# khanhptnk/magical-1

Hardware: AMD Instinct MI355X
Metric: env-steps/sec (whole node) at N instances/GPU, 1/2/4/8 MI355X (higher is better)
Workload: dtype f64

## Files before the change

magical-1_amd/csrc/mg_step.h:

```cpp
#pragma once
#include "mg_phys.h"
#include "mg_prof.h"

struct BodyR { int b; double minv, iinv; };
MG_DEV BodyR bodyr(const MGState &S, int e, int b) {
    if (b < 0) return {b, 0.0, 0.0};
    return {b, AT(S.bminv, b), AT(S.biinv, b)};
}
MG_DEV V2 bv(const MGState &S, int e, int b) { return b < 0 ? v2(0.0, 0.0) : v2(AT(S.bvx, b), AT(S.bvy, b)); }
MG_DEV double bwv(const MGState &S, int e, int b) { return b < 0 ? 0.0 : AT(S.bw, b); }
MG_DEV V2 bvb(const MGState &S, int e, int b) { return b < 0 ? v2(0.0, 0.0) : v2(AT(S.bvbx, b), AT(S.bvby, b)); }
MG_DEV double bwb(const MGState &S, int e, int b) { return b < 0 ? 0.0 : AT(S.bwb, b); }
MG_DEV V2 bp(const MGState &S, int e, int b) { return b < 0 ? v2(0.0, 0.0) : v2(AT(S.bpx, b), AT(S.bpy, b)); }
MG_DEV double ban(const MGState &S, int e, int b) { return b < 0 ? 0.0 : AT(S.ba, b); }

MG_DEV void apply_impulse(const MGState &S, int e, const BodyR &B, V2 j, V2 r) {
    if (B.b < 0) return;
    AT(S.bvx, B.b) = AT(S.bvx, B.b) + j.x * B.minv;
    AT(S.bvy, B.b) = AT(S.bvy, B.b) + j.y * B.minv;
    AT(S.bw, B.b) += B.iinv * vcross(r, j);
}
MG_DEV void apply_impulses(const MGState &S, int e, const BodyR &A, const BodyR &B, V2 r1, V2 r2, V2 j) {
    apply_impulse(S, e, A, vneg(j), r1);
    apply_impulse(S, e, B, j, r2);
// ... 227 lines not shown
    AT(S.au, slot) = u_a * u_b;
    AT(S.asa, slot) = sa_body; AT(S.asb, slot) = sb_body;
    if (AT(S.astate, slot) == ARB_CACHED) AT(S.astate, slot) = ARB_FIRST;
    int na_ = S.nactive[e];
    if (na_ < S.arb_cap) { AT(S.active, na_) = slot; S.nactive[e] = na_ + 1; }
    else S.overflow[e] |= 1;
    AT(S.astamp, slot) = S.stamp[e];
}

MG_DEV void arbiter_update(const MGState &S, const mg_library *L, int e, int key, const ShapeW &A, const ShapeW &B,
                           double ua, double ub, const Collision &info) {
    arbiter_update_t(S, L, e, key, A.type, A.body, B.type, B.body, ua, ub, info);
}

MG_DEV void arbiter_prestep(const MGState &S, const mg_library *L, int e, int slot, double dt) {
    int a = AT(S.asa, slot), b = AT(S.asb, slot);
    BodyR A = bodyr(S, e, a), B = bodyr(S, e, b);
    V2 n = v2(AT(S.anx, slot), AT(S.any, slot));
    V2 body_delta = vsub(bp(S, e, b), bp(S, e, a));
    int cnt = AT(S.acount, slot);
    for (int k = 0; k < cnt; k++) {
        V2 r1 = v2(ACON(k, AC_R1X, slot), ACON(k, AC_R1Y, slot)), r2 = v2(ACON(k, AC_R2X, slot), ACON(k, AC_R2Y, slot));
        ACON(k, AC_NMASS, slot) = 1.0 / (k_scalar_body(A, r1, n) + k_scalar_body(B, r2, n));
        V2 pn = vperp(n);
        ACON(k, AC_TMASS, slot) = 1.0 / (k_scalar_body(A, r1, pn) + k_scalar_body(B, r2, pn));
        double dist = vdot(vadd(vsub(r2, r1), body_delta), n);
        ACON(k, AC_BIAS, slot) = -L->collision_bias_coef * cpmin(0.0, dist + L->slop) / dt;
        ACON(k, AC_JB, slot) = 0.0;
    }
}

MG_DEV void arbiter_cached(const MGState &S, int e, int slot, double dt_coef) {
    if (AT(S.astate, slot) == ARB_FIRST) return;
    int a = AT(S.asa, slot), b = AT(S.asb, slot);
    BodyR A = bodyr(S, e, a), B = bodyr(S, e, b);
    V2 n = v2(AT(S.anx, slot), AT(S.any, slot));
    int cnt = AT(S.acount, slot);
    for (int k = 0; k < cnt; k++) {
        V2 j = vrotate(n, v2(ACON(k, AC_JN, slot), ACON(k, AC_JT, slot)));
        apply_impulses(S, e, A, B, v2(ACON(k, AC_R1X, slot), ACON(k, AC_R1Y, slot)),
                       v2(ACON(k, AC_R2X, slot), ACON(k, AC_R2Y, slot)), vmult(j, dt_coef));
    }
}

MG_DEV void arbiter_apply(const MGState &S, int e, int slot) {
    int a = AT(S.asa, slot), b = AT(S.asb, slot);
    BodyR A = bodyr(S, e, a), B = bodyr(S, e, b);
    V2 n = v2(AT(S.anx, slot), AT(S.any, slot));
    double friction = AT(S.au, slot);
    int cnt = AT(S.acount, slot);
    for (int k = 0; k < cnt; k++) {
        double nMass = ACON(k, AC_NMASS, slot);
        V2 r1 = v2(ACON(k, AC_R1X, slot), ACON(k, AC_R1Y, slot)), r2 = v2(ACON(k, AC_R2X, slot), ACON(k, AC_R2Y, slot));
        V2 vb1 = vadd(bvb(S, e, a), vmult(vperp(r1), bwb(S, e, a)));
        V2 vb2 = vadd(bvb(S, e, b), vmult(vperp(r2), bwb(S, e, b)));
        V2 vr = relative_velocity(S, e, a, b, r1, r2);
        double vbn = vdot(vsub(vb2, vb1), n);
        double vrn = vdot(vr, n);
        double vrt = vdot(vr, vperp(n));
        double jbn = (ACON(k, AC_BIAS, slot) - vbn) * nMass;
        double jbnOld = ACON(k, AC_JB, slot);
        double jBias = cpmax(jbnOld + jbn, 0.0);
        ACON(k, AC_JB, slot) = jBias;
        double jn = -(0.0 + vrn) * nMass;
        double jnOld = ACON(k, AC_JN, slot);
        double jnAcc = cpmax(jnOld + jn, 0.0);
        ACON(k, AC_JN, slot) = jnAcc;
        double jtMax = friction * jnAcc;
        double jt = -vrt * ACON(k, AC_TMASS, slot);
        double jtOld = ACON(k, AC_JT, slot);
        double jtAcc = cpclamp(jtOld + jt, -jtMax, jtMax);
        ACON(k, AC_JT, slot) = jtAcc;
        V2 jb = vmult(n, jBias - jbnOld);
        apply_bias_impulse(S, e, A, vneg(jb), r1);
        apply_bias_impulse(S, e, B, jb, r2);
        apply_impulses(S, e, A, B, r1, r2, vrotate(n, v2(jnAcc - jnOld, jtAcc - jtOld)));
    }
}

template <int NB>
struct RegBodies { double vx[NB], vy[NB], w[NB], vbx[NB], vby[NB], wb[NB], minv[NB], iinv[NB]; };

struct RegCons {
    double r1x, r1y, r2x, r2y, k11, k12, k21, k22, bias, bias2, jacc, jacc2, jmax, ratio, ratio_inv, isum, rate, twrn,
        wcoef;
};

template <int NB>
MG_DEV void rapply(RegBodies<NB> &R, int b, V2 j, V2 r) {
    if (b < 0) return;
    R.vx[b] = R.vx[b] + j.x * R.minv[b];
    R.vy[b] = R.vy[b] + j.y * R.minv[b];
    R.w[b] += R.iinv[b] * vcross(r, j);
}
template <int NB> MG_DEV V2 rv(const RegBodies<NB> &R, int b) { return b < 0 ? v2(0.0, 0.0) : v2(R.vx[b], R.vy[b]); }
template <int NB> MG_DEV double rw(const RegBodies<NB> &R, int b) { return b < 0 ? 0.0 : R.w[b]; }
template <int NB> MG_DEV double rii(const RegBodies<NB> &R, int b) { return b < 0 ? 0.0 : R.iinv[b]; }

template <int NB>
MG_DEV void rb_load(RegBodies<NB> &R, const MGState &S, int e) {
#pragma unroll
    for (int b = 0; b < NB; b++) {
        R.vx[b] = AT(S.bvx, b); R.vy[b] = AT(S.bvy, b); R.w[b] = AT(S.bw, b);
        R.vbx[b] = AT(S.bvbx, b); R.vby[b] = AT(S.bvby, b); R.wb[b] = AT(S.bwb, b);
        R.minv[b] = AT(S.bminv, b); R.iinv[b] = AT(S.biinv, b);
    }
}
template <int NB>
MG_DEV void rb_store(const RegBodies<NB> &R, const MGState &S, int e) {
#pragma unroll
    for (int b = 0; b < NB; b++) {
        AT(S.bvx, b) = R.vx[b]; AT(S.bvy, b) = R.vy[b]; AT(S.bw, b) = R.w[b];
        AT(S.bvbx, b) = R.vbx[b]; AT(S.bvby, b) = R.vby[b]; AT(S.bwb, b) = R.wb[b];
    }
}

MG_DEV void rc_load(RegCons &q, const MGState &S, int e, int c, int type, double dt) {
    q.jacc = CPA(CP_JACC, c); q.jacc2 = 0.0; q.jmax = CPA(CP_MAXF, c) * dt;
    q.isum = CPA(CP_ISUM, c); q.bias = CPA(CP_BIAS, c);
    if (type == MG_C_PIVOT) {
        q.jacc2 = CPA(CP_JACC2, c); q.bias2 = CPA(CP_BIAS2, c);
        q.r1x = CPA(CP_R1X, c); q.r1y = CPA(CP_R1Y, c); q.r2x = CPA(CP_R2X, c); q.r2y = CPA(CP_R2Y, c);
        q.k11 = CPA(CP_K11, c); q.k12 = CPA(CP_K12, c); q.k21 = CPA(CP_K21, c); q.k22 = CPA(CP_K22, c);
    }
    if (type == MG_C_GEAR) { q.ratio = CPA(CP_RATIO, c); q.ratio_inv = CPA(CP_RATIO_INV, c); }
    if (type == MG_C_MOTOR) q.rate = CPA(CP_RATE, c);
    if (type == MG_C_SPRING) { q.twrn = CPA(CP_TWRN, c); q.wcoef = CPA(CP_WCOEF, c); }
}
MG_DEV void rc_store(const RegCons &q, const MGState &S, int e, int c, int type) {
    CPA(CP_JACC, c) = q.jacc;
    if (type == MG_C_PIVOT) CPA(CP_JACC2, c) = q.jacc2;
    if (type == MG_C_SPRING) CPA(CP_TWRN, c) = q.twrn;
}

template <int NB>
MG_DEV void rcons_cached(RegBodies<NB> &R, const RegCons &q, int a, int b, int type, double dt_coef) {
    switch (type) {
    case MG_C_PIVOT: {
        V2 j = vmult(v2(q.jacc, q.jacc2), dt_coef);
        rapply(R, a, vneg(j), v2(q.r1x, q.r1y));
        rapply(R, b, j, v2(q.r2x, q.r2y));
        break;
    }
    case MG_C_GEAR: {
        double j = q.jacc * dt_coef;
        if (a >= 0) R.w[a] -= j * R.iinv[a] * q.ratio_inv;
        if (b >= 0) R.w[b] += j * R.iinv[b];
        break;
    }
    case MG_C_ROTLIMIT:
    case MG_C_MOTOR: {
        double j = q.jacc * dt_coef;
        if (a >= 0) R.w[a] -= j * R.iinv[a];
        if (b >= 0) R.w[b] += j * R.iinv[b];
        break;
    }
    default: break;
    }
}

template <int NB>
MG_DEV void rcons_apply(RegBodies<NB> &R, RegCons &q, int a, int b, int type) {
    switch (type) {
    case MG_C_PIVOT: {
        V2 r1 = v2(q.r1x, q.r1y), r2 = v2(q.r2x, q.r2y);
        V2 v1 = vadd(rv(R, a), vmult(vperp(r1), rw(R, a)));
        V2 v2_ = vadd(rv(R, b), vmult(vperp(r2), rw(R, b)));
        V2 vr = vsub(v2_, v1);
        V2 d = vsub(v2(q.bias, q.bias2), vr);
        V2 j = v2(d.x * q.k11 + d.y * q.k12, d.x * q.k21 + d.y * q.k22);
        V2 jOld = v2(q.jacc, q.jacc2);
        V2 jAcc = vclamp(vadd(jOld, j), q.jmax);
        q.jacc = jAcc.x; q.jacc2 = jAcc.y;
        V2 dj = vsub(jAcc, jOld);
        rapply(R, a, vneg(dj), r1);
        rapply(R, b, dj, r2);
        break;
    }
    case MG_C_GEAR: {
        double wr = rw(R, b) * q.ratio - rw(R, a);
        double j = (q.bias - wr) * q.isum;
        double jOld = q.jacc;
        double jAcc = cpclamp(jOld + j, -q.jmax, q.jmax);
        q.jacc = jAcc;
        j = jAcc - jOld;
        if (a >= 0) R.w[a] -= j * R.iinv[a] * q.ratio_inv;
        if (b >= 0) R.w[b] += j * R.iinv[b];
        break;
    }
    case MG_C_ROTLIMIT: {
        double bias = q.bias;
        if (!bias) return;
        double wr = rw(R, b) - rw(R, a);
        double j = -(bias + wr) * q.isum;
        double jOld = q.jacc;
        double jAcc = bias < 0.0 ? cpclamp(jOld + j, 0.0, q.jmax) : cpclamp(jOld + j, -q.jmax, 0.0);
        q.jacc = jAcc;
        j = jAcc - jOld;
        if (a >= 0) R.w[a] -= j * R.iinv[a];
        if (b >= 0) R.w[b] += j * R.iinv[b];
        break;
    }
    case MG_C_MOTOR: {
        double wr = rw(R, b) - rw(R, a) + q.rate;
        double j = -wr * q.isum;
        double jOld = q.jacc;
        double jAcc = cpclamp(jOld + j, -q.jmax, q.jmax);
        q.jacc = jAcc;
        j = jAcc - jOld;
        if (a >= 0) R.w[a] -= j * R.iinv[a];
        if (b >= 0) R.w[b] += j * R.iinv[b];
        break;
    }
    case MG_C_SPRING: {
        double wrn = rw(R, a) - rw(R, b);
        double w_damp = (q.twrn - wrn) * q.wcoef;
        q.twrn = wrn + w_damp;
        double j_damp = w_damp * q.isum;
        q.jacc += j_damp;
        if (a >= 0) R.w[a] += j_damp * R.iinv[a];
        if (b >= 0) R.w[b] -= j_damp * R.iinv[b];
        break;
    }
    }
}

__host__ __device__ constexpr bool shape_body_slot(int k) { return k == 0 || k == 4 || k == 5 || k == 6; }
template <int NB>
struct ArbBody { bool m[NB]; };
template <int NB>
MG_DEV ArbBody<NB> arb_body(int b) {
    ArbBody<NB> h;
#pragma unroll
    for (int k = 0; k < NB; k++) h.m[k] = shape_body_slot(k) && b == k;
    return h;
}
template <int NB>
MG_DEV double hsel(const double (&x)[NB], const ArbBody<NB> &h) {
    double r = 0.0;
#pragma unroll
    for (int k = 0; k < NB; k++)
        if (shape_body_slot(k)) r = h.m[k] ? x[k] : r;
    return r;
}
template <int NB>
MG_DEV void hput(double (&x)[NB], const ArbBody<NB> &h, double v) {
#pragma unroll
    for (int k = 0; k < NB; k++)
        if (shape_body_slot(k)) x[k] = h.m[k] ? v : x[k];
}
template <int NB>
MG_DEV void happly(RegBodies<NB> &R, const ArbBody<NB> &h, double minv, double iinv, V2 j, V2 r) {
    hput(R.vx, h, hsel(R.vx, h) + j.x * minv);
    hput(R.vy, h, hsel(R.vy, h) + j.y * minv);
    hput(R.w, h, hsel(R.w, h) + iinv * vcross(r, j));
}
template <int NB>
MG_DEV void happly_bias(RegBodies<NB> &R, const ArbBody<NB> &h, double minv, double iinv, V2 j, V2 r) {
    hput(R.vbx, h, hsel(R.vbx, h) + j.x * minv);
    hput(R.vby, h, hsel(R.vby, h) + j.y * minv);
    hput(R.wb, h, hsel(R.wb, h) + iinv * vcross(r, j));
}
template <int NB>
MG_DEV void harb_cached(RegBodies<NB> &R, const MGState &S, int e, int slot, double dt_coef) {
    if (AT(S.astate, slot) == ARB_FIRST) return;
    const ArbBody<NB> ha = arb_body<NB>(AT(S.asa, slot)), hb = arb_body<NB>(AT(S.asb, slot));
    const double am = hsel(R.minv, ha), ai = hsel(R.iinv, ha), bm = hsel(R.minv, hb), bi = hsel(R.iinv, hb);
    V2 n = v2(AT(S.anx, slot), AT(S.any, slot));
    int cnt = AT(S.acount, slot);
    for (int k = 0; k < cnt; k++) {
        V2 j = vmult(vrotate(n, v2(ACON(k, AC_JN, slot), ACON(k, AC_JT, slot))), dt_coef);
        happly(R, ha, am, ai, vneg(j), v2(ACON(k, AC_R1X, slot), ACON(k, AC_R1Y, slot)));
        happly(R, hb, bm, bi, j, v2(ACON(k, AC_R2X, slot), ACON(k, AC_R2Y, slot)));
    }
}
template <int NB>
MG_DEV void harb_apply(RegBodies<NB> &R, const MGState &S, int e, int slot) {
    const int sa = AT(S.asa, slot), sb = AT(S.asb, slot);
    const ArbBody<NB> ha = arb_body<NB>(sa), hb = arb_body<NB>(sb);
    const double am = hsel(R.minv, ha), ai = hsel(R.iinv, ha), bm = hsel(R.minv, hb), bi = hsel(R.iinv, hb);
    const bool wa = __ballot(sa >= 0) != 0, wb = __ballot(sb >= 0) != 0;
    V2 n = v2(AT(S.anx, slot), AT(S.any, slot));
    double friction = AT(S.au, slot);
    int cnt = AT(S.acount, slot);
    for (int k = 0; k < cnt; k++) {
        double nMass = ACON(k, AC_NMASS, slot);
        V2 r1 = v2(ACON(k, AC_R1X, slot), ACON(k, AC_R1Y, slot)), r2 = v2(ACON(k, AC_R2X, slot), ACON(k, AC_R2Y, slot));
        V2 vb1 = v2(0.0, 0.0), v1 = v2(0.0, 0.0), vb2 = v2(0.0, 0.0), v2_ = v2(0.0, 0.0);
        if (wa) {
            vb1 = vadd(v2(hsel(R.vbx, ha), hsel(R.vby, ha)), vmult(vperp(r1), hsel(R.wb, ha)));
            v1 = vadd(v2(hsel(R.vx, ha), hsel(R.vy, ha)), vmult(vperp(r1), hsel(R.w, ha)));
        }
        if (wb) {
            vb2 = vadd(v2(hsel(R.vbx, hb), hsel(R.vby, hb)), vmult(vperp(r2), hsel(R.wb, hb)));
            v2_ = vadd(v2(hsel(R.vx, hb), hsel(R.vy, hb)), vmult(vperp(r2), hsel(R.w, hb)));
        }
        V2 vr = vsub(v2_, v1);
        double vbn = vdot(vsub(vb2, vb1), n);
        double vrn = vdot(vr, n);
        double vrt = vdot(vr, vperp(n));
        double jbn = (ACON(k, AC_BIAS, slot) - vbn) * nMass;
        double jbnOld = ACON(k, AC_JB, slot);
// ... 154 lines not shown
        if (k < a.cnt) { ACON(k, AC_JB, slot) = a.jb[k]; ACON(k, AC_JN, slot) = a.jn[k]; ACON(k, AC_JT, slot) = a.jt[k]; }
}
template <int NB, int A, int B>
MG_DEV void rarb_apply_k(RegBodies<NB> &R, RegArb &a) {
    const double am = A >= 0 ? R.minv[A] : 0.0, ai = A >= 0 ? R.iinv[A] : 0.0;
    const double bm = B >= 0 ? R.minv[B] : 0.0, bi = B >= 0 ? R.iinv[B] : 0.0;
    const V2 n = v2(a.nx, a.ny);
#pragma unroll
    for (int k = 0; k < 2; k++) {
        if (k >= a.cnt) break;
        const double nMass = a.nm[k];
        V2 r1 = v2(a.r1x[k], a.r1y[k]), r2 = v2(a.r2x[k], a.r2y[k]);
        V2 vb1 = v2(0.0, 0.0), v1 = v2(0.0, 0.0), vb2 = v2(0.0, 0.0), v2_ = v2(0.0, 0.0);
        if constexpr (A >= 0) {
            vb1 = vadd(v2(R.vbx[A], R.vby[A]), vmult(vperp(r1), R.wb[A]));
            v1 = vadd(v2(R.vx[A], R.vy[A]), vmult(vperp(r1), R.w[A]));
        }
        if constexpr (B >= 0) {
            vb2 = vadd(v2(R.vbx[B], R.vby[B]), vmult(vperp(r2), R.wb[B]));
            v2_ = vadd(v2(R.vx[B], R.vy[B]), vmult(vperp(r2), R.w[B]));
        }
        V2 vr = vsub(v2_, v1);
        double vbn = vdot(vsub(vb2, vb1), n);
        double vrn = vdot(vr, n);
        double vrt = vdot(vr, vperp(n));
        double jbn = (a.bias[k] - vbn) * nMass;
        double jbnOld = a.jb[k];
        double jBias = cpmax(jbnOld + jbn, 0.0);
        a.jb[k] = jBias;
        double jn = -(0.0 + vrn) * nMass;
        double jnOld = a.jn[k];
        double jnAcc = cpmax(jnOld + jn, 0.0);
        a.jn[k] = jnAcc;
        double jtMax = a.fr * jnAcc;
        double jt = -vrt * a.tm[k];
        double jtOld = a.jt[k];
        double jtAcc = cpclamp(jtOld + jt, -jtMax, jtMax);
        a.jt[k] = jtAcc;
        V2 jb = vmult(n, jBias - jbnOld);
        if constexpr (A >= 0) {
            const V2 m = vneg(jb);
            R.vbx[A] = R.vbx[A] + m.x * am; R.vby[A] = R.vby[A] + m.y * am; R.wb[A] = R.wb[A] + ai * vcross(r1, m);
        }
        if constexpr (B >= 0) {
            R.vbx[B] = R.vbx[B] + jb.x * bm; R.vby[B] = R.vby[B] + jb.y * bm; R.wb[B] = R.wb[B] + bi * vcross(r2, jb);
        }
        V2 j = vrotate(n, v2(jnAcc - jnOld, jtAcc - jtOld));
        if constexpr (A >= 0) {
            const V2 m = vneg(j);
            R.vx[A] = R.vx[A] + m.x * am; R.vy[A] = R.vy[A] + m.y * am; R.w[A] = R.w[A] + ai * vcross(r1, m);
        }
        if constexpr (B >= 0) {
            R.vx[B] = R.vx[B] + j.x * bm; R.vy[B] = R.vy[B] + j.y * bm; R.w[B] = R.w[B] + bi * vcross(r2, j);
        }
    }
}
template <int NB>
MG_DEV void rarb_row(RegBodies<NB> &R, RegArb &a) {
    switch (a.code) {
    case 0: rarb_apply_k<NB, 0, -1>(R, a); break;
    case 1: rarb_apply_k<NB, -1, 4>(R, a); break;
    case 2: rarb_apply_k<NB, -1, 5>(R, a); break;
    default:
        if constexpr (NB > 6) {
            switch (a.code) {
            case 3: rarb_apply_k<NB, -1, 6>(R, a); break;
            case 4: rarb_apply_k<NB, 0, 6>(R, a); break;
            case 5: rarb_apply_k<NB, 4, 6>(R, a); break;
            default: rarb_apply_k<NB, 5, 6>(R, a); break;
            }
        }
        break;
    }
}

template <int NCS, int C = 0>
MG_DEV void rstatic_load(RegCons *q, const MGState &S, int e, double dt) {
    if constexpr (C < NCS) {
        rc_load(q[C], S, e, C, static_cons(C).type, dt);
        rstatic_load<NCS, C + 1>(q, S, e, dt);
    }
}
template <int NCS, int C = 0>
MG_DEV void rstatic_store(const RegCons *q, const MGState &S, int e) {
    if constexpr (C < NCS) {
        rc_store(q[C], S, e, C, static_cons(C).type);
        rstatic_store<NCS, C + 1>(q, S, e);
    }
}
template <int NCS, int NB, int C = 0>
MG_DEV void rstatic_cached(RegBodies<NB> &R, const RegCons *q, double dt_coef) {
    if constexpr (C < NCS) {
        constexpr ConsDesc d = static_cons(C);
        rcons_cached(R, q[C], d.a, d.b, d.type, dt_coef);
        rstatic_cached<NCS, NB, C + 1>(R, q, dt_coef);
    }
}
template <int NCS, int NB, int C = 0>
MG_DEV void rstatic_apply(RegBodies<NB> &R, RegCons *q) {
    if constexpr (C < NCS) {
        constexpr ConsDesc d = static_cons(C);
        rcons_apply(R, q[C], d.a, d.b, d.type);
        rstatic_apply<NCS, NB, C + 1>(R, q);
    }
}

__host__ __device__ constexpr int static_nbodies(int ncs) { return ncs > 10 ? 7 : 6; }

template <int NCS, int NARB>
MG_DEV void static_solve(const MGState &S, int e, double dt, double dt_coef, int nact, MGProf &P) {
    constexpr int NB = static_nbodies(NCS);
    RegBodies<NB> R;
    RegCons q[NCS];
    rb_load(R, S, e);
    rstatic_load<NCS>(q, S, e, dt);
    for (int i = 0; i < nact; i++) harb_cached_row(R, S, e, AT(S.active, i), dt_coef);
    rstatic_cached<NCS>(R, q, dt_coef);
    MG_PP(P, 5);
    RegArb ra[NARB > 0 ? NARB : 1];
    int nreg = 0;
    if constexpr (NARB > 0) {
#pragma unroll
        for (int i = 0; i < NARB; i++) {
            ra[i].code = -1; ra[i].cnt = 0;
            if (i < nact) rarb_load(ra[i], S, e, AT(S.active, i));
        }
        bool ok = true;
#pragma unroll
        for (int i = 0; i < NARB; i++) {
            if (i < nact && ok && ra[i].code >= 0 && (NB > 6 || ra[i].code <= 2)) nreg = i + 1;
            else ok = false;
        }
    }
#pragma unroll 1
    for (int it = 0; it < MG_ITERATIONS; it++) {
        if constexpr (NARB > 0) {
#pragma unroll
            for (int i = 0; i < NARB; i++)
                if (i < nreg) rarb_row(R, ra[i]);
        }
        for (int i = nreg; i < nact; i++) harb_row(R, S, e, AT(S.active, i));
        rstatic_apply<NCS>(R, q);
    }
    if constexpr (NARB > 0) {
#pragma unroll
        for (int i = 0; i < NARB; i++)
            if (i < nreg) rarb_store(ra[i], S, e, AT(S.active, i));
    }
    rb_store(R, S, e);
    rstatic_store<NCS>(q, S, e);
}

MG_DEV void space_step(const MGState &S, const mg_library *L, int e, double dt, MGProf &P) {
    uint32_t stamp = S.stamp[e] + 1;
    S.stamp[e] = stamp;
    double prev_dt = S.curr_dt[e];
    S.curr_dt[e] = dt;
    int nact = S.nactive[e];
    for (int i = 0; i < nact; i++) AT(S.astate, AT(S.active, i)) = ARB_NORMAL;
    S.nactive[e] = 0;
    int nb = S.nbodies[e];
    for (int b = 0; b < nb; b++) {
        AT(S.bpx, b) = AT(S.bpx, b) + (AT(S.bvx, b) + AT(S.bvbx, b)) * dt;
        AT(S.bpy, b) = AT(S.bpy, b) + (AT(S.bvy, b) + AT(S.bvby, b)) * dt;
        body_set_angle_step(S, e, b, AT(S.ba, b) + (AT(S.bw, b) + AT(S.bwb, b)) * dt);
        AT(S.bvbx, b) = 0.0; AT(S.bvby, b) = 0.0; AT(S.bwb, b) = 0.0;
    }
    int ns = S.nshapes[e];
    for (int k = 0; k < ns; k++) shape_update_bb(S, L, e, k);
    MG_PP(P, 1);
    ShapeW A, W, B;
    for (int i = 0; i < ns; i++) {
        const double al = AT(S.sbbl, i), ab = AT(S.sbbb, i), ar = AT(S.sbbr, i), at = AT(S.sbbt, i);
        bool have_a = false;
        const int gi = AT(S.sgroup, i), bi = AT(S.sbody, i);
        const double ui = AT(S.su, i);
        for (int w = 0; w < 4 && !(gi & MG_GROUP_OFF); w++) {
            double wl, wb, wr, wt;
            wall_bb(w, wl, wb, wr, wt);
            if (!(al <= wr && wl <= ar && ab <= wt && wb <= at)) continue;
            if (!have_a) { load_shape(S, L, e, i, (uint64_t)AT(S.shash, i), A); have_a = true; }
            load_wall(w, W);
            Collision info;
            collide(A, W, info);
            if (info.count) arbiter_update(S, L, e, i * 128 + 100 + w, A, W, ui, 0.8, info);
        }
        for (int j = i + 1; j < ns; j++) {
            if (!(al <= AT(S.sbbr, j) && AT(S.sbbl, j) <= ar && ab <= AT(S.sbbt, j) && AT(S.sbbb, j) <= at))
                continue;
            if (AT(S.sbody, j) == bi) continue;
            int gj = AT(S.sgroup, j);
            if ((gi != 0 && gi == gj) || ((gi | gj) & MG_GROUP_OFF)) continue;
            if (surely_apart(S, L, e, i, j)) continue;
            if (!have_a) { load_shape(S, L, e, i, (uint64_t)AT(S.shash, i), A); have_a = true; }
            load_shape(S, L, e, j, (uint64_t)AT(S.shash, j), B);
            Collision info;
            collide(A, B, info);
            if (info.count) arbiter_update(S, L, e, i * 128 + j, A, B, ui, AT(S.su, j), info);
        }
    }
    MG_PP(P, 2);
    for (int i = 0; i < S.arb_cap; i++) {
        if (AT(S.akey, i) < 0) continue;
        uint32_t ticks = stamp - AT(S.astamp, i);
        if (ticks >= 1 && AT(S.astate, i) != ARB_CACHED) AT(S.astate, i) = ARB_CACHED;
        if (ticks >= 3) { AT(S.akey, i) = -1; AT(S.acount, i) = 0; }
    }
    MG_PP(P, 3);
    nact = S.nactive[e];
    int nc = S.ncons[e];
    for (int i = 0; i < nact; i++) arbiter_prestep(S, L, e, AT(S.active, i), dt);
    for (int c = 0; c < nc; c++) cons_prestep(S, e, c, dt);
    MG_PP(P, 4);
    double dt_coef = (prev_dt == 0.0 ? 0.0 : dt / prev_dt);
    for (int i = 0; i < nact; i++) arbiter_cached(S, e, AT(S.active, i), dt_coef);
    for (int c = 0; c < nc; c++) cons_cached(S, e, c, dt_coef);
    MG_PP(P, 5);
    for (int it = 0; it < MG_ITERATIONS; it++) {
        for (int i = 0; i < nact; i++) arbiter_apply(S, e, AT(S.active, i));
        for (int c = 0; c < nc; c++) cons_apply(S, e, c, dt);
    }
    MG_PP(P, 6);
}

MG_DEV double rl_d(double v, int src) {
    const uint64_t u = (uint64_t)__double_as_longlong(v);
    const uint32_t lo = (uint32_t)__builtin_amdgcn_readlane((int)(uint32_t)u, src);
    const uint32_t hi = (uint32_t)__builtin_amdgcn_readlane((int)(uint32_t)(u >> 32), src);
    return __longlong_as_double((long long)(((uint64_t)hi << 32) | lo));
}
MG_DEV uint64_t rl_u64(uint64_t v, int src) {
    const uint32_t lo = (uint32_t)__builtin_amdgcn_readlane((int)(uint32_t)v, src);
    const uint32_t hi = (uint32_t)__builtin_amdgcn_readlane((int)(uint32_t)(v >> 32), src);
// ... 736 lines not shown
```

magical-1_amd/csrc/mg_stepq.h:

```cpp
#pragma once
#include "mg_step.h"

template <int QL> MG_DEV int qlane(int ev, int s) { return ev * QL + s; }

MG_DEV double qshfl(double v, int src) {
    const uint64_t u = __double_as_longlong(v);
    const uint32_t lo = (uint32_t)__shfl((int)(uint32_t)u, src, 64), hi = (uint32_t)__shfl((int)(uint32_t)(u >> 32), src, 64);
    return __longlong_as_double((long long)(((uint64_t)hi << 32) | lo));
}
MG_DEV uint64_t qshfl_u64(uint64_t u, int src) {
    const uint32_t lo = (uint32_t)__shfl((int)(uint32_t)u, src, 64), hi = (uint32_t)__shfl((int)(uint32_t)(u >> 32), src, 64);
    return ((uint64_t)hi << 32) | lo;
}

template <int NC, int QL, int C = 0>
MG_DEV void static_prestep_quad(const MGState &S, int e, int sub, double dt) {
    if constexpr (C < NC) {
        constexpr ConsDesc d = static_cons(C);
        constexpr int owner = d.type == MG_C_SPRING ? 0 : C % QL;
        if (sub == owner) cons_prestep_impl(S, e, C, d.a, d.b, d.type, dt);
        static_prestep_quad<NC, QL, C + 1>(S, e, sub, dt);
    }
}

MG_DEV int quad_body(int p, int nb) {
    if (p == 0) return 0;
    if (p == 1) return 4;
    if (p == 2) return 5;
    if (nb == 7) return p == 3 ? 6 : p - 3;
    return p - 2;
}

MG_DEV uint64_t qshfl_xor_u64(uint64_t u, int m) {
    const uint32_t lo = (uint32_t)__shfl_xor((int)(uint32_t)u, m, 64), hi = (uint32_t)__shfl_xor((int)(uint32_t)(u >> 32), m, 64);
    return ((uint64_t)hi << 32) | lo;
}

MG_DEV bool quad_candidate(const MGState &S, const mg_library *L, int e, int i, int k) {
    const double al = AT(S.sbbl, i), ab = AT(S.sbbb, i), ar = AT(S.sbbr, i), at = AT(S.sbbt, i);
    const int gi = AT(S.sgroup, i);
    if (k < 4) {
        if (gi & MG_GROUP_OFF) return false;
        double wl, wb, wr, wt;
        wall_bb(k, wl, wb, wr, wt);
        return al <= wr && wl <= ar && ab <= wt && wb <= at;
    }
    const int j = i + 1 + (k - 4), gj = AT(S.sgroup, j);
    return al <= AT(S.sbbr, j) && AT(S.sbbl, j) <= ar && ab <= AT(S.sbbt, j) && AT(S.sbbb, j) <= at &&
           AT(S.sbody, j) != AT(S.sbody, i) && !((gi != 0 && gi == gj) || ((gi | gj) & MG_GROUP_OFF)) &&
           !surely_apart(S, L, e, i, j);
}

template <int NCS, int QL>
MG_DEV void narrowphase_quad(const MGState &S, const mg_library *L, int e, int sub, int ns) {
    ShapeW A, B;
    const int ntot = 4 * ns + (ns * (ns - 1)) / 2;
    for (int w0 = 0; w0 < ntot; w0 += 64) {
        const int wn = ntot - w0 < 64 ? ntot - w0 : 64;
        uint64_t hits = 0;
        {
            int i = 0, k = w0 + sub;
            while (i < ns && k >= 4 + ns - 1 - i) { k -= 4 + ns - 1 - i; i++; }
            for (int c = sub; c < wn; c += QL) {
                if (quad_candidate(S, L, e, i, k)) hits |= 1ull << c;
                k += QL;
                while (i < ns && k >= 4 + ns - 1 - i) { k -= 4 + ns - 1 - i; i++; }
            }
        }
#pragma unroll
        for (int off = 1; off < QL; off <<= 1)
            hits |= qshfl_xor_u64(hits, off);
        while (hits) {
            uint64_t rest = hits;
            int mine = -1;
#pragma unroll
            for (int q = 0; q < QL; q++) {
                if (!rest) break;
                const int b = __ffsll((long long)rest) - 1;
                rest &= rest - 1;
                if (q == sub) mine = b;
            }
            hits = rest;
            Collision info;
            info.count = 0;
            int key = 0, ta = 0, bi = 0, tb = 0, bb = -1;
            double ui = 0.0, ub = 0.0;
            if (mine >= 0) {
                int i = 0, k = w0 + mine;
                while (k >= 4 + ns - 1 - i) { k -= 4 + ns - 1 - i; i++; }
                bi = AT(S.sbody, i); ui = AT(S.su, i);
                ta = AT(S.spoly, i) < 0 ? WS_CIRCLE : WS_POLY;
                load_shape(S, L, e, i, (uint64_t)AT(S.shash, i), A);
                if (k < 4) {
                    load_wall(k, B);
                    key = i * 128 + 100 + k; ub = 0.8; tb = WS_SEGMENT; bb = -1;
                } else {
                    const int j = i + 1 + (k - 4);
                    load_shape(S, L, e, j, (uint64_t)AT(S.shash, j), B);
                    key = i * 128 + j; ub = AT(S.su, j); tb = B.type; bb = B.body;
                }
                collide(A, B, info);
            }
            const uint64_t bal = __ballot(info.count > 0);
            uint32_t m = 0;
#pragma unroll
            for (int s = 0; s < QL; s++) m |= (uint32_t)((bal >> qlane<QL>(e, s)) & 1ull) << s;
            for (int s = 0; s < QL; s++) {
                if (!((m >> s) & 1u)) continue;
                const int src = qlane<QL>(e, s);
                Collision q;
                q.count = __shfl(info.count, src, 64);
                q.n = v2(qshfl(info.n.x, src), qshfl(info.n.y, src));
#pragma unroll
                for (int kk = 0; kk < 2; kk++) {
                    q.p1[kk] = v2(qshfl(info.p1[kk].x, src), qshfl(info.p1[kk].y, src));
                    q.p2[kk] = v2(qshfl(info.p2[kk].x, src), qshfl(info.p2[kk].y, src));
                    q.hash[kk] = qshfl_u64(info.hash[kk], src);
                }
                const int qkey = __shfl(key, src, 64), qta = __shfl(ta, src, 64), qbi = __shfl(bi, src, 64);
                const int qtb = __shfl(tb, src, 64), qbb = __shfl(bb, src, 64);
                const double qui = qshfl(ui, src), qub = qshfl(ub, src);
                if (sub == 0) arbiter_update_t(S, L, e, qkey, qta, qbi, qtb, qbb, qui, qub, q);
            }
        }
    }
}

template <int NCS, int QL>
MG_DEV void space_step_quad(const MGState &S, const mg_library *L, int e, int sub, double dt, MGProf &P) {
    __syncthreads();
    const double prev_dt = S.curr_dt[e];
    const uint32_t stamp = S.stamp[e] + 1;
    const int nact0 = S.nactive[e], nb = S.nbodies[e], ns = S.nshapes[e];
    for (int i = sub; i < nact0; i += QL) AT(S.astate, AT(S.active, i)) = ARB_NORMAL;
    for (int p = sub; p < nb; p += QL) {
        const int b = quad_body(p, nb);
        AT(S.bpx, b) = AT(S.bpx, b) + (AT(S.bvx, b) + AT(S.bvbx, b)) * dt;
        AT(S.bpy, b) = AT(S.bpy, b) + (AT(S.bvy, b) + AT(S.bvby, b)) * dt;
        body_set_angle_step(S, e, b, AT(S.ba, b) + (AT(S.bw, b) + AT(S.bwb, b)) * dt);
        AT(S.bvbx, b) = 0.0; AT(S.bvby, b) = 0.0; AT(S.bwb, b) = 0.0;
    }
    __syncthreads();
    if (sub == 0) { S.stamp[e] = stamp; S.curr_dt[e] = dt; S.nactive[e] = 0; }
    for (int k = sub; k < ns; k += QL) shape_update_bb(S, L, e, k);
    __syncthreads();
    MG_PP(P, 1);
    narrowphase_quad<NCS, QL>(S, L, e, sub, ns);
    __syncthreads();
    MG_PP(P, 2);
    for (int i = sub; i < S.arb_cap; i += QL) {
        if (AT(S.akey, i) < 0) continue;
        const uint32_t ticks = stamp - AT(S.astamp, i);
        if (ticks >= 1 && AT(S.astate, i) != ARB_CACHED) AT(S.astate, i) = ARB_CACHED;
        if (ticks >= 3) { AT(S.akey, i) = -1; AT(S.acount, i) = 0; }
    }
    __syncthreads();
    MG_PP(P, 3);
    const int nact = S.nactive[e];
    for (int i = sub; i < nact; i += QL) arbiter_prestep(S, L, e, AT(S.active, i), dt);
    static_prestep_quad<NCS, QL>(S, e, sub, dt);
    __syncthreads();
    MG_PP(P, 4);
    const double dt_coef = (prev_dt == 0.0 ? 0.0 : dt / prev_dt);
    if (sub == 0) static_solve<NCS, (QL >= 8 ? 1 : 0)>(S, e, dt, dt_coef, nact, P);
    MG_PP(P, 6);
}

template <int NCS, int QL>
__device__ __forceinline__ void env_substeps_quad(const MGState &V, const mg_library *L, int ev, int sub, int a,
                                                  MGProf &P) {
    __syncthreads();
    if (sub == 0) {
        robot_set_action(V, L, ev, a < 18 ? a : 0);
        robot_update<true>(V, L, ev);
    }
    const double dt = L->dt;
    for (int i = 0; i < 10; i++) {
        MG_PP(P, 0);
        space_step_quad<NCS, QL>(V, L, ev, sub, dt, P);
        if (sub == 0 && i < 9) robot_update<true>(V, L, ev);
    }
    __syncthreads();
}
```

Before: 3.488 million.

## Stream static constraint params per iteration instead of holding all in registers

Splits per-constraint state into read-only parameters (RegCons) and accumulators (RegAcc). For quad layouts with QL>=8, the solver now reloads constraint parameters from memory one constraint ahead while iterating, instead of keeping the whole array in registers. For larger constraint counts it also streams the accumulators through memory on each iteration. This aims to cut register pressure and spills in the single-lane static solve, at the cost of repeated global or cache loads and stores inside the iteration loop.

```diff
diff --git a/magical-1_amd/csrc/mg_step.h b/magical-1_amd/csrc/mg_step.h
--- a/magical-1_amd/csrc/mg_step.h
+++ b/magical-1_amd/csrc/mg_step.h
@@ -333,9 +333,9 @@
 struct RegBodies { double vx[NB], vy[NB], w[NB], vbx[NB], vby[NB], wb[NB], minv[NB], iinv[NB]; };
 
 struct RegCons {
-    double r1x, r1y, r2x, r2y, k11, k12, k21, k22, bias, bias2, jacc, jacc2, jmax, ratio, ratio_inv, isum, rate, twrn,
-        wcoef;
+    double r1x, r1y, r2x, r2y, k11, k12, k21, k22, bias, bias2, jmax, ratio, ratio_inv, isum, rate, wcoef;
 };
+struct RegAcc { double jacc, jacc2, twrn; };
 
 template <int NB>
 MG_DEV void rapply(RegBodies<NB> &R, int b, V2 j, V2 r) {
@@ -367,41 +367,47 @@
 }
 
 MG_DEV void rc_load(RegCons &q, const MGState &S, int e, int c, int type, double dt) {
-    q.jacc = CPA(CP_JACC, c); q.jacc2 = 0.0; q.jmax = CPA(CP_MAXF, c) * dt;
+    q = RegCons{};
+    q.jmax = CPA(CP_MAXF, c) * dt;
     q.isum = CPA(CP_ISUM, c); q.bias = CPA(CP_BIAS, c);
     if (type == MG_C_PIVOT) {
-        q.jacc2 = CPA(CP_JACC2, c); q.bias2 = CPA(CP_BIAS2, c);
+        q.bias2 = CPA(CP_BIAS2, c);
         q.r1x = CPA(CP_R1X, c); q.r1y = CPA(CP_R1Y, c); q.r2x = CPA(CP_R2X, c); q.r2y = CPA(CP_R2Y, c);
         q.k11 = CPA(CP_K11, c); q.k12 = CPA(CP_K12, c); q.k21 = CPA(CP_K21, c); q.k22 = CPA(CP_K22, c);
     }
     if (type == MG_C_GEAR) { q.ratio = CPA(CP_RATIO, c); q.ratio_inv = CPA(CP_RATIO_INV, c); }
     if (type == MG_C_MOTOR) q.rate = CPA(CP_RATE, c);
-    if (type == MG_C_SPRING) { q.twrn = CPA(CP_TWRN, c); q.wcoef = CPA(CP_WCOEF, c); }
-}
-MG_DEV void rc_store(const RegCons &q, const MGState &S, int e, int c, int type) {
-    CPA(CP_JACC, c) = q.jacc;
-    if (type == MG_C_PIVOT) CPA(CP_JACC2, c) = q.jacc2;
-    if (type == MG_C_SPRING) CPA(CP_TWRN, c) = q.twrn;
+    if (type == MG_C_SPRING) q.wcoef = CPA(CP_WCOEF, c);
+}
+MG_DEV void ra_load(RegAcc &j, const MGState &S, int e, int c, int type) {
+    j.jacc = CPA(CP_JACC, c); j.jacc2 = 0.0; j.twrn = 0.0;
+    if (type == MG_C_PIVOT) j.jacc2 = CPA(CP_JACC2, c);
+    if (type == MG_C_SPRING) j.twrn = CPA(CP_TWRN, c);
+}
+MG_DEV void ra_store(const RegAcc &j, const MGState &S, int e, int c, int type) {
+    CPA(CP_JACC, c) = j.jacc;
+    if (type == MG_C_PIVOT) CPA(CP_JACC2, c) = j.jacc2;
+    if (type == MG_C_SPRING) CPA(CP_TWRN, c) = j.twrn;
 }
 
 template <int NB>
-MG_DEV void rcons_cached(RegBodies<NB> &R, const RegCons &q, int a, int b, int type, double dt_coef) {
+MG_DEV void rcons_cached(RegBodies<NB> &R, const RegCons &q, const RegAcc &acc, int a, int b, int type, double dt_coef) {
     switch (type) {
     case MG_C_PIVOT: {
-        V2 j = vmult(v2(q.jacc, q.jacc2), dt_coef);
+        V2 j = vmult(v2(acc.jacc, acc.jacc2), dt_coef);
         rapply(R, a, vneg(j), v2(q.r1x, q.r1y));
         rapply(R, b, j, v2(q.r2x, q.r2y));
         break;
     }
     case MG_C_GEAR: {
-        double j = q.jacc * dt_coef;
+        double j = acc.jacc * dt_coef;
         if (a >= 0) R.w[a] -= j * R.iinv[a] * q.ratio_inv;
         if (b >= 0) R.w[b] += j * R.iinv[b];
         break;
     }
     case MG_C_ROTLIMIT:
     case MG_C_MOTOR: {
-        double j = q.jacc * dt_coef;
+        double j = acc.jacc * dt_coef;
         if (a >= 0) R.w[a] -= j * R.iinv[a];
         if (b >= 0) R.w[b] += j * R.iinv[b];
         break;
@@ -411,7 +417,7 @@
 }
 
 template <int NB>
-MG_DEV void rcons_apply(RegBodies<NB> &R, RegCons &q, int a, int b, int type) {
+MG_DEV void rcons_apply(RegBodies<NB> &R, const RegCons &q, RegAcc &acc, int a, int b, int type) {
     switch (type) {
     case MG_C_PIVOT: {
         V2 r1 = v2(q.r1x, q.r1y), r2 = v2(q.r2x, q.r2y);
@@ -420,9 +426,9 @@
         V2 vr = vsub(v2_, v1);
         V2 d = vsub(v2(q.bias, q.bias2), vr);
         V2 j = v2(d.x * q.k11 + d.y * q.k12, d.x * q.k21 + d.y * q.k22);
-        V2 jOld = v2(q.jacc, q.jacc2);
+        V2 jOld = v2(acc.jacc, acc.jacc2);
         V2 jAcc = vclamp(vadd(jOld, j), q.jmax);
-        q.jacc = jAcc.x; q.jacc2 = jAcc.y;
+        acc.jacc = jAcc.x; acc.jacc2 = jAcc.y;
         V2 dj = vsub(jAcc, jOld);
         rapply(R, a, vneg(dj), r1);
         rapply(R, b, dj, r2);
@@ -431,9 +437,9 @@
     case MG_C_GEAR: {
         double wr = rw(R, b) * q.ratio - rw(R, a);
         double j = (q.bias - wr) * q.isum;
-        double jOld = q.jacc;
+        double jOld = acc.jacc;
         double jAcc = cpclamp(jOld + j, -q.jmax, q.jmax);
-        q.jacc = jAcc;
+        acc.jacc = jAcc;
         j = jAcc - jOld;
         if (a >= 0) R.w[a] -= j * R.iinv[a] * q.ratio_inv;
         if (b >= 0) R.w[b] += j * R.iinv[b];
@@ -444,9 +450,9 @@
         if (!bias) return;
         double wr = rw(R, b) - rw(R, a);
         double j = -(bias + wr) * q.isum;
-        double jOld = q.jacc;
+        double jOld = acc.jacc;
         double jAcc = bias < 0.0 ? cpclamp(jOld + j, 0.0, q.jmax) : cpclamp(jOld + j, -q.jmax, 0.0);
-        q.jacc = jAcc;
+        acc.jacc = jAcc;
         j = jAcc - jOld;
         if (a >= 0) R.w[a] -= j * R.iinv[a];
         if (b >= 0) R.w[b] += j * R.iinv[b];
@@ -455,9 +461,9 @@
     case MG_C_MOTOR: {
         double wr = rw(R, b) - rw(R, a) + q.rate;
         double j = -wr * q.isum;
-        double jOld = q.jacc;
+        double jOld = acc.jacc;
         double jAcc = cpclamp(jOld + j, -q.jmax, q.jmax);
-        q.jacc = jAcc;
+        acc.jacc = jAcc;
         j = jAcc - jOld;
         if (a >= 0) R.w[a] -= j * R.iinv[a];
         if (b >= 0) R.w[b] += j * R.iinv[b];
@@ -465,10 +471,10 @@
     }
     case MG_C_SPRING: {
         double wrn = rw(R, a) - rw(R, b);
-        double w_damp = (q.twrn - wrn) * q.wcoef;
-        q.twrn = wrn + w_damp;
+        double w_damp = (acc.twrn - wrn) * q.wcoef;
+        acc.twrn = wrn + w_damp;
         double j_damp = w_damp * q.isum;
-        q.jacc += j_damp;
+        acc.jacc += j_damp;
         if (a >= 0) R.w[a] += j_damp * R.iinv[a];
         if (b >= 0) R.w[b] -= j_damp * R.iinv[b];
         break;
@@ -789,40 +795,85 @@
     }
 }
 template <int NCS, int C = 0>
-MG_DEV void rstatic_store(const RegCons *q, const MGState &S, int e) {
+MG_DEV void rstatic_load_acc(RegAcc *acc, const MGState &S, int e) {
     if constexpr (C < NCS) {
-        rc_store(q[C], S, e, C, static_cons(C).type);
-        rstatic_store<NCS, C + 1>(q, S, e);
+        ra_load(acc[C], S, e, C, static_cons(C).type);
+        rstatic_load_acc<NCS, C + 1>(acc, S, e);
+    }
+}
+template <int NCS, int C = 0>
+MG_DEV void rstatic_store(const RegAcc *acc, const MGState &S, int e) {
+    if constexpr (C < NCS) {
+        ra_store(acc[C], S, e, C, static_cons(C).type);
+        rstatic_store<NCS, C + 1>(acc, S, e);
     }
 }
 template <int NCS, int NB, int C = 0>
-MG_DEV void rstatic_cached(RegBodies<NB> &R, const RegCons *q, double dt_coef) {
+MG_DEV void rstatic_cached(RegBodies<NB> &R, const RegCons *q, const RegAcc *acc, double dt_coef) {
     if constexpr (C < NCS) {
         constexpr ConsDesc d = static_cons(C);
-        rcons_cached(R, q[C], d.a, d.b, d.type, dt_coef);
-        rstatic_cached<NCS, NB, C + 1>(R, q, dt_coef);
+        rcons_cached(R, q[C], acc[C], d.a, d.b, d.type, dt_coef);
+        rstatic_cached<NCS, NB, C + 1>(R, q, acc, dt_coef);
     }
 }
 template <int NCS, int NB, int C = 0>
-MG_DEV void rstatic_apply(RegBodies<NB> &R, RegCons *q) {
+MG_DEV void rstatic_apply(RegBodies<NB> &R, const RegCons *q, RegAcc *acc) {
     if constexpr (C < NCS) {
         constexpr ConsDesc d = static_cons(C);
-        rcons_apply(R, q[C], d.a, d.b, d.type);
-        rstatic_apply<NCS, NB, C + 1>(R, q);
+        rcons_apply(R, q[C], acc[C], d.a, d.b, d.type);
+        rstatic_apply<NCS, NB, C + 1>(R, q, acc);
+    }
+}
+
+template <int NCS, int NB, int C = 0>
+MG_DEV void rstream_cached(RegBodies<NB> &R, RegCons &cur, const RegAcc *acc, const MGState &S, int e, double dt,
+                           double dt_coef) {
+    if constexpr (C < NCS) {
+        constexpr ConsDesc d = static_cons(C);
+        constexpr int N = (C + 1) % NCS;
+        RegCons nxt;
+        rc_load(nxt, S, e, N, static_cons(N).type, dt);
+        rcons_cached(R, cur, acc[C], d.a, d.b, d.type, dt_coef);
+        cur = nxt;
+        rstream_cached<NCS, NB, C + 1>(R, cur, acc, S, e, dt, dt_coef);
+    }
+}
+template <int NCS, int NB, bool ACCW, int C = 0>
+MG_DEV void rstream_apply(RegBodies<NB> &R, RegCons &cur, RegAcc *acc, const MGState &S, int e, double dt) {
+    if constexpr (C < NCS) {
+        constexpr ConsDesc d = static_cons(C);
+        constexpr int N = (C + 1) % NCS;
+        RegCons nxt;
+        RegAcc nacc;
+        rc_load(nxt, S, e, N, static_cons(N).type, dt);
+        if constexpr (ACCW) {
+            ra_load(nacc, S, e, N, static_cons(N).type);
+            rcons_apply(R, cur, acc[0], d.a, d.b, d.type);
+            ra_store(acc[0], S, e, C, d.type);
+            acc[0] = nacc;
+        } else {
+            rcons_apply(R, cur, acc[C], d.a, d.b, d.type);
+        }
+        cur = nxt;
+        rstream_apply<NCS, NB, ACCW, C + 1>(R, cur, acc, S, e, dt);
     }
 }
 
 __host__ __device__ constexpr int static_nbodies(int ncs) { return ncs > 10 ? 7 : 6; }
 
-template <int NCS, int NARB>
+template <int NCS, int NARB, int STREAM>
 MG_DEV void static_solve(const MGState &S, int e, double dt, double dt_coef, int nact, MGProf &P) {
     constexpr int NB = static_nbodies(NCS);
     RegBodies<NB> R;
-    RegCons q[NCS];
+    RegCons q[STREAM ? 1 : NCS];
+    RegAcc acc[NCS];
     rb_load(R, S, e);
-    rstatic_load<NCS>(q, S, e, dt);
+    if constexpr (STREAM) rc_load(q[0], S, e, 0, static_cons(0).type, dt);
+    else rstatic_load<NCS>(q, S, e, dt);
+    rstatic_load_acc<NCS>(acc, S, e);
     for (int i = 0; i < nact; i++) harb_cached_row(R, S, e, AT(S.active, i), dt_coef);
-    rstatic_cached<NCS>(R, q, dt_coef);
+    if constexpr (STREAM) rstream_cached<NCS>(R, q[0], acc, S, e, dt, dt_coef);
+    else rstatic_cached<NCS>(R, q, acc, dt_coef);
     MG_PP(P, 5);
     RegArb ra[NARB > 0 ? NARB : 1];
     int nreg = 0;
@@ -847,7 +898,9 @@
                 if (i < nreg) rarb_row(R, ra[i]);
         }
         for (int i = nreg; i < nact; i++) harb_row(R, S, e, AT(S.active, i));
-        rstatic_apply<NCS>(R, q);
+        if constexpr (STREAM == 2) rstream_apply<NCS, NB, true>(R, q[0], acc, S, e, dt);
+        else if constexpr (STREAM) rstream_apply<NCS, NB, false>(R, q[0], acc, S, e, dt);
+        else rstatic_apply<NCS>(R, q, acc);
     }
     if constexpr (NARB > 0) {
 #pragma unroll
@@ -855,7 +908,7 @@
             if (i < nreg) rarb_store(ra[i], S, e, AT(S.active, i));
     }
     rb_store(R, S, e);
-    rstatic_store<NCS>(q, S, e);
+    if constexpr (STREAM != 2) rstatic_store<NCS>(acc, S, e);
 }
 
 MG_DEV void space_step(const MGState &S, const mg_library *L, int e, double dt, MGProf &P) {
diff --git a/magical-1_amd/csrc/mg_stepq.h b/magical-1_amd/csrc/mg_stepq.h
--- a/magical-1_amd/csrc/mg_stepq.h
+++ b/magical-1_amd/csrc/mg_stepq.h
@@ -1,5 +1,7 @@
 #pragma once
 #include "mg_step.h"
+
+__host__ __device__ constexpr int quad_stream(int ncs, int ql) { return ql < 8 ? 0 : ncs > 10 ? 2 : 1; }
 
 template <int QL> MG_DEV int qlane(int ev, int s) { return ev * QL + s; }
 
@@ -162,7 +164,7 @@
     __syncthreads();
     MG_PP(P, 4);
     const double dt_coef = (prev_dt == 0.0 ? 0.0 : dt / prev_dt);
-    if (sub == 0) static_solve<NCS, (QL >= 8 ? 1 : 0)>(S, e, dt, dt_coef, nact, P);
+    if (sub == 0) static_solve<NCS, (QL >= 8 ? 1 : 0), quad_stream(NCS, QL)>(S, e, dt, dt_coef, nact, P);
     MG_PP(P, 6);
 }
 
```

After: 3.551 million, median of 6. 1.02x the previous value.
